# HicrestLaboratory/DLNetBench

Hardware: AMD Instinct MI355X
Metric: proxy iter time (ms) + effective GB/s, Llama-3-8B DP/FSDP at 1/2/4/8 MI355X (lower is better)
Workload: dtype bf16

## Files before the change

csrc/include/dlnb/kernels.hpp:

```cpp
#pragma once

#include <cstddef>
#include <cstdint>

#include "dlnb/common.hpp"

namespace dlnb {
namespace kernels {

void fill_random(void* p, size_t count, DType t, uint64_t seed, void* stream);

enum DlCounter : int {
  kCappedTasks = 0,
  kCappedTicks = 1,
  kWaitTimeouts = 2,
  kGateTimeouts = 3,
  kAbsorbedTicks = 4,
  kAbsorbedTasks = 5,
  kAborted = 6,
  kLateBlocks = 7,
  kNumCounters = 8
};
constexpr uint64_t kPoisonIter = ~0ull;
struct DlSync {
  uint64_t* tstart[2] = {nullptr, nullptr};
  const uint64_t* gate[2] = {nullptr, nullptr};
  uint32_t tag[2] = {0, 0};
  uint32_t chain = 0;
  uint64_t* counters = nullptr;
  const uint64_t* iter = nullptr;
  uint64_t gate_timeout = 0;
  uint64_t* done_gate = nullptr;
  uint32_t done_tag = 0;
  uint32_t pad = 0;
  const uint64_t* abort = nullptr;
};
constexpr uint32_t kTaskGateOnly = 1;
struct DlTask {
  DlSync sync;
  uint64_t ticks = 0;
  uint32_t epoch = 0;
  uint32_t work_rounds = 0;
  uint32_t tail_kt = 0;
  uint32_t flags = 0;
  uint64_t* tend = nullptr;
};
void gate_signal(uint64_t* gate, const uint64_t* iter, uint32_t tag, void* stream);
void fail_gate_signal(long index);
void gate_wait(const uint64_t* gate, const uint64_t* iter, uint32_t tag, uint64_t timeout_ticks, uint64_t* timeouts,
               void* stream, const uint64_t* abort = nullptr);
void set_word(uint64_t* word, uint64_t value, void* stream);
bool queues_independent(void* a, void* b, uint64_t timeout_ticks);

void idle_wait(uint64_t ticks, void* stream, uint64_t* start = nullptr, uint64_t* start2 = nullptr);
void busy_spin(uint64_t ticks, int blocks, void* stream, uint64_t* start = nullptr, uint64_t* start2 = nullptr);
double wallclock_hz(int device);
double wallclock_hz_nominal(int device);
double wallclock_uncertainty_ppm(int device);
void clock_cal_begin(int device);
void stamp(uint64_t* slot, void* stream);
void host_signal(uint64_t* word, uint64_t value, void* stream);
void lane_done(uint64_t* word, const uint64_t* iter, void* stream);
void host_wait(const uint64_t* word, uint64_t value, uint64_t timeout_ticks, uint64_t* timeouts, void* stream,
               uint64_t* iter_out = nullptr, uint64_t iter_value = 0, const uint64_t* abort = nullptr);
int num_cus(int device);

bool gemm_shape_ok(int M, int N, int K, DType in_t);
void gemm_tn(const void* A, const void* B, void* C, int M, int N, int K, int lda, int ldb, int ldc, DType in_t,
             void* stream, int variant = 0);
bool gemm_8phase_shape_ok(int M, int N, int K, DType in_t);
bool gemm_4wave_fp8_shape_ok(int M, int N, int K, DType in_t);
int gemm_group();
int gemm_narrow_nf(int M, int N, int cus);
bool gemm_tn_narrow(const void* A, const void* B, void* C, int M, int N, int K, int lda, int ldb, int ldc,
                    DType in_t, void* stream);
void gemm_tn_4wave_fp8(const void* A, const void* B, void* C, int M, int N, int K, int lda, int ldb, int ldc,
                       void* stream);
bool gemm_4wave_shape_ok(int M, int N, int K, DType in_t);
void gemm_tn_4wave_bf16(const void* A, const void* B, void* C, int M, int N, int K, int lda, int ldb, int ldc,
                        void* stream);
void gemm_tn_4wave_deadline(const void* A, const void* B, void* C, int M, int N, int K, DType in_t, uint64_t ticks,
                            uint64_t* slot, uint32_t epoch, int grid, void* stream, uint64_t slice_end,
                            const DlSync& sync);
void gemm_tn_4wave_fp8_deadline(const void* A, const void* B, void* C, int M, int N, int K, uint64_t ticks,
                                uint64_t* slot, uint32_t epoch, int grid, void* stream, uint64_t slice_end,
                                const DlSync& sync);
void gemm_tn_8phase(const void* A, const void* B, void* C, int M, int N, int K, int lda, int ldb, int ldc, DType in_t,
                    void* stream);
void gemm_tn_8phase_deadline(const void* A, const void* B, void* C, int M, int N, int K, DType in_t, uint64_t ticks,
                             uint64_t* slot, uint32_t epoch, int grid, void* stream, uint64_t slice_end,
                             const DlSync& sync);

void gemm_tn_deadline(const void* A, const void* B, void* C, int M, int N, int K, DType in_t, uint64_t ticks,
                      uint64_t* slot, uint32_t epoch, int grid, void* stream, uint64_t slice_end = 0,
                      const DlSync& sync = DlSync());

bool deadline_program_ok(int M, int N, int K, DType in_t);
void gemm_tn_deadline_program(const void* A, const void* B, void* C, int M, int N, int K, DType in_t,
                              const DlTask* tasks, int n, uint64_t* slot, int grid, void* stream,
                              uint32_t epoch = 0);
int program_ktiles(int M, int N, int K, DType in_t);
int program_tail_multiple(int M, int N, int K, DType in_t);

void sgd_momentum_bf16(void* param, void* mom, const void* grad, size_t n, float lr, float beta, void* stream,
                       uint64_t* end_stamp = nullptr, uint32_t* done = nullptr);

}
}
```

csrc/kernels/gemm_8phase.hip:

```cpp
#include <hip/hip_runtime.h>

#include <cstdlib>

#include "deadline_sync.hpp"
#include "dlnb/kernels.hpp"
#include "store_pair.hpp"

namespace dlnb {
namespace kernels {

namespace {

typedef __attribute__((ext_vector_type(8))) __bf16 bf16x8;
typedef __attribute__((ext_vector_type(4))) __bf16 bf16x4;
typedef __attribute__((ext_vector_type(4))) float f32x4;
typedef __attribute__((ext_vector_type(8))) int i32x8;
typedef __attribute__((ext_vector_type(4))) int i32x4;
typedef __attribute__((address_space(3))) void* lds_ptr_t;
typedef __attribute__((address_space(1))) void* gbl_ptr_t;

constexpr int kT = 256;
constexpr int kRB = 128;
constexpr int kHalf = 128 * kRB;
constexpr int kBuf = 4 * kHalf;
enum : int { kA0 = 0, kA1 = 1, kB0 = 2, kB1 = 3 };

__device__ __forceinline__ int swz(int row, int chunk) { return row * kRB + ((chunk ^ ((row >> 1) & 7)) << 4); }

template <int N>
__device__ __forceinline__ void wait_vm() {
  static_assert(N >= 0 && N < 64, "vmcnt range");
  __builtin_amdgcn_s_waitcnt((N & 15) | ((N >> 4) << 14) | (7 << 4) | (15 << 8));
}

__device__ __forceinline__ void raw_barrier() {
  __builtin_amdgcn_sched_barrier(0);
  __builtin_amdgcn_s_barrier();
  __builtin_amdgcn_sched_barrier(0);
}

__device__ __forceinline__ void stage_half(const char* base, int voff, size_t ld, int soff, char* lds, int w) {
  const __amdgpu_buffer_rsrc_t rs = __builtin_amdgcn_make_buffer_rsrc(const_cast<char*>(base), 0, 0x7ffffff0, 0x00020000);
#pragma unroll
  for (int i = 0; i < 2; ++i)
    __builtin_amdgcn_raw_ptr_buffer_load_lds(rs, (lds_ptr_t)(lds + (i * 8 + w) * 1024), 16, voff,
                                             soff + i * 64 * static_cast<int>(ld), 0, 0);
}

__device__ __forceinline__ int lane_offset(size_t ld, int w, int lane) {
  const int slot = w * 64 + lane;
  const int r = slot >> 3;
  const int q = (slot & 7) ^ ((r >> 1) & 7);
  return static_cast<int>(r * ld) + (q << 4);
}

__device__ __forceinline__ int xcd_remap(int b, int T) {
  const int q = T / 8, r = T % 8, x = b % 8;
  return (x < r ? x * (q + 1) : r * (q + 1) + (x - r) * q) + b / 8;
}

template <bool FP8>
struct Frags;
template <>
struct Frags<false> {
  bf16x8 a[2][4], bx[2][2], by[2][2];
};
template <>
struct Frags<true> {
  i32x8 a[4], bx[2], by[2];
};

template <bool FP8, int NF>
__device__ __forceinline__ void read_frags(const char* half, int row0, int r16, int h, bf16x8 (&f)[2][NF]) {
#pragma unroll
  for (int ks = 0; ks < 2; ++ks)
#pragma unroll
    for (int i = 0; i < NF; ++i) f[ks][i] = *reinterpret_cast<const bf16x8*>(half + swz(row0 + i * 16 + r16, ks * 4 + h));
}
template <bool FP8, int NF>
__device__ __forceinline__ void read_frags(const char* half, int row0, int r16, int h, i32x8 (&f)[NF]) {
#pragma unroll
  for (int i = 0; i < NF; ++i) {
    const int row = row0 + i * 16 + r16;
    const i32x4 lo = *reinterpret_cast<const i32x4*>(half + swz(row, h));
    const i32x4 hi = *reinterpret_cast<const i32x4*>(half + swz(row, h + 4));
    f[i] = __builtin_shufflevector(lo, hi, 0, 1, 2, 3, 4, 5, 6, 7);
  }
}

__device__ __forceinline__ void mfma_quadrant(f32x4 (&acc)[4][2], const bf16x8 (&a)[2][4], const bf16x8 (&b)[2][2]) {
#pragma unroll
  for (int ks = 0; ks < 2; ++ks)
#pragma unroll
    for (int i = 0; i < 4; ++i)
#pragma unroll
      for (int j = 0; j < 2; ++j) acc[i][j] = __builtin_amdgcn_mfma_f32_16x16x32_bf16(b[ks][j], a[ks][i], acc[i][j], 0, 0, 0);
}
__device__ __forceinline__ void mfma_quadrant(f32x4 (&acc)[4][2], const i32x8 (&a)[4], const i32x8 (&b)[2]) {
#pragma unroll
  for (int i = 0; i < 4; ++i)
#pragma unroll
    for (int j = 0; j < 2; ++j)
      acc[i][j] = __builtin_amdgcn_mfma_scale_f32_16x16x128_f8f6f4(b[j], a[i], acc[i][j], 0, 0, 0, 127, 0, 127);
}

struct Ctx {
  const char* Ab;
  const char* Bb;
  size_t lda, ldb;
  char* smem;
  int w, lane, wr, wc, r16, h;
  int last_kt;
  int voffA, voffB;
};

__device__ __forceinline__ void stage(const Ctx& c, int t, int slot) {
  const int tk = min(t, c.last_kt);
  const bool isA = slot == kA0 || slot == kA1;
  const int hi = slot == kA1 || slot == kB1;
  const char* base = isA ? c.Ab + static_cast<size_t>(hi) * 128 * c.lda : c.Bb + static_cast<size_t>(hi) * 128 * c.ldb;
  stage_half(base, isA ? c.voffA : c.voffB, isA ? c.lda : c.ldb, tk * kRB, c.smem + (t & 1) * kBuf + slot * kHalf, c.w);
}

typedef __attribute__((address_space(3))) volatile int lds_flag_t;
struct Deadline {
  uint64_t t0, ticks, slice_end;
  lds_flag_t* flag;
  int tid;
};

template <bool FP8, bool DL, bool BAL, int Q, int VM, bool STAGE, typename AF, typename BF>
__device__ __forceinline__ bool phase(const Ctx& c, int v, AF& fa, BF& b0r, BF& b1r, f32x4 (&acc)[2][2][4][2],
                                      const Deadline& d, uint64_t& now, bool has_next) {
  const char* cur = c.smem + (v & 1) * kBuf;
  if constexpr (Q == 0) {
    if constexpr (!BAL) {
      read_frags<FP8, 2>(cur + kB0 * kHalf, c.wc * 32, c.r16, c.h, b0r);
      __builtin_amdgcn_sched_barrier(0);
    }
    read_frags<FP8, 4>(cur + kA0 * kHalf, c.wr * 64, c.r16, c.h, fa);
  } else if constexpr (Q == 1) {
    read_frags<FP8, 2>(cur + kB1 * kHalf, c.wc * 32, c.r16, c.h, b1r);
  } else if constexpr (Q == 2) {
    read_frags<FP8, 4>(cur + kA1 * kHalf, c.wr * 64, c.r16, c.h, fa);
  } else {
    if constexpr (DL) {
      if (d.tid == 0) {
        const uint64_t el = (now - d.t0) & ((1ull << 48) - 1);
        d.flag[v & 1] = el >= d.ticks || el >= d.slice_end;
        asm volatile("s_waitcnt lgkmcnt(0)" ::: "memory");
      }
    }
    if constexpr (BAL) {
      if (has_next) read_frags<FP8, 2>(c.smem + ((v + 1) & 1) * kBuf + kB0 * kHalf, c.wc * 32, c.r16, c.h, b1r);
    }
  }
  if constexpr (STAGE) {
    if constexpr (Q == 0) stage(c, v + 1, kB1);
    if constexpr (Q == 1) stage(c, v + 1, kA1);
    if constexpr (Q == 2) stage(c, v + 2, BAL ? kB0 : kA0);
    if constexpr (Q == 3) stage(c, v + 2, BAL ? kA0 : kB0);
  }
  wait_vm<VM>();
  raw_barrier();
  int flag = 0;
  if constexpr (DL && Q == 3) flag = d.flag[v & 1];
  __builtin_amdgcn_sched_barrier(0);
  __builtin_amdgcn_s_setprio(1);
  if constexpr (Q == 0) mfma_quadrant(acc[0][0], fa, b0r);
  if constexpr (Q == 1) mfma_quadrant(acc[0][1], fa, b1r);
  if constexpr (Q == 2) mfma_quadrant(acc[1][1], fa, b1r);
  if constexpr (Q == 3) mfma_quadrant(acc[1][0], fa, b0r);
  __builtin_amdgcn_s_setprio(0);
  __builtin_amdgcn_sched_barrier(0);
  if constexpr (DL && Q == 2) now = __builtin_amdgcn_s_memrealtime();
  bool stop = false;
  if constexpr (DL && Q == 3) stop = __builtin_amdgcn_readfirstlane(flag) != 0;
  raw_barrier();
  return stop;
}

template <bool FP8, bool DL, bool BAL, int PAR, int V0, int V1, int V2, int V3, bool S01, bool S23>
__device__ __forceinline__ bool ktile(const Ctx& c, int v, Frags<FP8>& f, f32x4 (&acc)[2][2][4][2], const Deadline& d,
                                      bool has_next = true) {
  uint64_t now = 0;
  auto& b0r = (BAL && PAR == 1) ? f.by : f.bx;
  auto& b1r = (BAL && PAR == 1) ? f.bx : f.by;
  phase<FP8, DL, BAL, 0, V0, S01>(c, v, f.a, b0r, b1r, acc, d, now, has_next);
  phase<FP8, DL, BAL, 1, V1, S01>(c, v, f.a, b0r, b1r, acc, d, now, has_next);
  phase<FP8, DL, BAL, 2, V2, S23>(c, v, f.a, b0r, b1r, acc, d, now, has_next);
  return phase<FP8, DL, BAL, 3, V3, S23>(c, v, f.a, b0r, b1r, acc, d, now, has_next);
}

template <bool FP8, bool DL, bool BAL, int PAR>
__device__ __forceinline__ bool tail(const Ctx& c, int v, Frags<FP8>& f, f32x4 (&acc)[2][2][4][2], const Deadline& d) {
  if (ktile<FP8, DL, BAL, PAR, 8, 8, 6, 4, true, false>(c, v, f, acc, d)) return true;
  return ktile<FP8, DL, BAL, 1 - PAR, 2, 0, 0, 0, false, false>(c, v + 1, f, acc, d, false);
}

template <bool FP8, bool DL, bool BAL, bool UNI = false>
__device__ __forceinline__ bool tile(Ctx& c, const char* __restrict__ A, const char* __restrict__ B,
                                     __bf16* __restrict__ C, int M, int N, int K, int ldc, int b, const Deadline& d,
                                     int GROUP = 8) {
  const int nt_m = M / kT, nt_n = N / kT;
  const int per_group = GROUP * nt_n;
  const int first_m = (b / per_group) * GROUP;
  const int gsz = min(nt_m - first_m, GROUP);
  const int tm = first_m + (b % per_group) % gsz;
  const int tn = (b % per_group) / gsz;
  constexpr int esz = FP8 ? 1 : 2;
  c.Ab = A + static_cast<size_t>(tm) * kT * c.lda;
  c.Bb = B + static_cast<size_t>(tn) * kT * c.ldb;
  const int nk = (K * esz) / kRB;
  c.last_kt = UNI ? nk - 1 : 1 << 30;

  f32x4 acc[2][2][4][2];
#pragma unroll
  for (int qm = 0; qm < 2; ++qm)
#pragma unroll
    for (int qn = 0; qn < 2; ++qn)
#pragma unroll
      for (int i = 0; i < 4; ++i)
#pragma unroll
        for (int j = 0; j < 2; ++j) acc[qm][qn][i][j] = f32x4{0.f, 0.f, 0.f, 0.f};
  Frags<FP8> f;

  stage(c, 0, BAL ? kB0 : kA0);
  stage(c, 0, BAL ? kA0 : kB0);
  stage(c, 0, kB1);
  stage(c, 0, kA1);
  stage(c, 1, BAL ? kB0 : kA0);
  stage(c, 1, BAL ? kA0 : kB0);
  wait_vm<8>();
  raw_barrier();
  if constexpr (BAL) read_frags<FP8, 2>(c.smem + kB0 * kHalf, c.wc * 32, c.r16, c.h, f.bx);
  if (c.wr == 1) raw_barrier();

  bool stop = false;
  int v = 0;
  if constexpr (UNI) {
    if constexpr (!BAL) {
      for (; v < nk && !stop; ++v) stop = ktile<FP8, DL, false, 0, 8, 8, 8, 8, true, true>(c, v, f, acc, d);
    } else {
      for (; v < nk && !stop; v += 2) {
        stop = ktile<FP8, DL, true, 0, 8, 8, 8, 8, true, true>(c, v, f, acc, d);
        if (!stop) stop = ktile<FP8, DL, true, 1, 8, 8, 8, 8, true, true>(c, v + 1, f, acc, d);
      }
    }
    wait_vm<0>();
  } else if constexpr (!BAL) {
    for (; v < nk - 2 && !stop; ++v) stop = ktile<FP8, DL, false, 0, 8, 8, 8, 8, true, true>(c, v, f, acc, d);
    if (!stop) stop = tail<FP8, DL, false, 0>(c, v, f, acc, d);
  } else {
    for (; v < nk - 2 && !stop; v += 2) {
      stop = ktile<FP8, DL, true, 0, 8, 8, 8, 8, true, true>(c, v, f, acc, d);
      if (!stop) stop = ktile<FP8, DL, true, 1, 8, 8, 8, 8, true, true>(c, v + 1, f, acc, d);
    }
    if (!stop) stop = tail<FP8, DL, true, 0>(c, v, f, acc, d);
  }
  if (c.wr == 0) raw_barrier();
  if constexpr (DL) {
    if (stop) {
      wait_vm<0>();
      return false;
    }
  }

  const bool wide = epi::wide_ok(C, ldc);
#pragma unroll
  for (int qm = 0; qm < 2; ++qm)
#pragma unroll
    for (int qn = 0; qn < 2; ++qn)
#pragma unroll
      for (int i = 0; i < 4; ++i) {
        const int m = tm * kT + qm * 128 + c.wr * 64 + i * 16 + c.r16;
        const int n = tn * kT + qn * 128 + c.wc * 32;
        epi::store_pair<DL>(C + static_cast<size_t>(m) * ldc + n, acc[qm][qn][i][0], acc[qm][qn][i][1], c.h, wide);
      }
  return true;
}

template <bool FP8, bool DL, bool BAL = false, bool UNI = false>
__global__ void __launch_bounds__(512, 1)
    gemm_8phase_kernel(const char* __restrict__ A, const char* __restrict__ B, __bf16* __restrict__ C, int M, int N,
                       int K, int lda, int ldb, int ldc, uint64_t* __restrict__ slot, uint32_t epoch, uint64_t ticks,
                       uint64_t slice_end, DlSync sync, int group = 8, const DlTask* __restrict__ prog = nullptr,
                       int ntasks = 0) {
  __shared__ __attribute__((aligned(16))) char smem[2 * kBuf + 16];
  const int tid = threadIdx.x;
  Ctx c;
  c.lane = tid & 63;
  c.w = __builtin_amdgcn_readfirstlane(tid >> 6);
  c.wr = c.w >> 2;
  c.wc = c.w & 3;
  c.r16 = c.lane & 15;
  c.h = c.lane >> 4;
  c.smem = smem;
  constexpr int esz = FP8 ? 1 : 2;
  c.lda = static_cast<size_t>(lda) * esz;
  c.ldb = static_cast<size_t>(ldb) * esz;
  c.voffA = lane_offset(c.lda, c.w, c.lane);
  c.voffB = lane_offset(c.ldb, c.w, c.lane);
  const int T = (M / kT) * (N / kT);
  Deadline d{0, ticks, slice_end, (lds_flag_t*)(smem + 2 * kBuf), tid};
  if constexpr (!DL) {
    tile<FP8, false, BAL, UNI>(c, A, B, C, M, N, K, ldc, xcd_remap(blockIdx.x, T), d, group);
  } else {
    int round = 0;
    for (int k = 0;; ++k) {
      bool fixed = false;
      if (prog) {
        d.ticks = d.slice_end = prog[k].ticks;
        fixed = d.ticks == 0 && (prog[k].work_rounds | prog[k].tail_kt | prog[k].flags) != 0;
        if (d.ticks == 0 && !fixed) {
          if (blockIdx.x == 0 && tid == 0)
            for (int j = k; j < ntasks; ++j) dl::join(prog[j].sync);
          return;
        }
      }
      if (tid == 0) {
        if (prog) {
          const dl::ProgSeq ps = dl::program_seq(prog, k, epoch);
          d.t0 = dl::start_task(slot, ps.seq, ps.ep16, ps.mono, d.ticks, prog[k].sync, ps.it, k > 0).t0;
        } else {
          d.t0 = dl::agree_t0(slot, epoch, ticks, sync);
        }
      }
      if (fixed) {
        d.ticks = d.slice_end = 1ull << 48;
        const int rounds = static_cast<int>(prog[k].work_rounds);
        for (int r = 0; r < rounds; ++r, ++round)
          tile<FP8, true, BAL, UNI>(c, A, B, C, M, N, K, ldc, xcd_remap((blockIdx.x + round * gridDim.x) % T, T), d);
        const int tkt = static_cast<int>(prog[k].tail_kt);
        if (tkt > 0) {
          tile<FP8, true, BAL, UNI>(c, A, B, C, M, N, tkt * kRB / esz, ldc,
                                    xcd_remap((blockIdx.x + round * gridDim.x) % T, T), d);
          ++round;
        }
        if (tid == 0) dl::fixed_done(slot, prog[k].sync, prog[k].tend);
        if (k + 1 >= ntasks) return;
        continue;
      }
      if (prog && (prog[k].flags & kTaskGateOnly)) {
        dl::task_done(prog[k].sync);
// ... 46 lines not shown

struct StreamCtx {
  const char* A;
  const char* B;
  int nt_m, nt_n, T, nk;
  const char *Ab0, *Ab1, *Bb0, *Bb1;
};

__device__ __forceinline__ void stage_g(const Ctx& c, const StreamCtx& sc, int t, int base, int slot) {
  const int nxt = t - base >= sc.nk;
  const int kt = t - base - nxt * sc.nk;
  const bool isA = slot == kA0 || slot == kA1;
  const int hi = slot == kA1 || slot == kB1;
  const char* ab = nxt ? sc.Ab1 : sc.Ab0;
  const char* bb = nxt ? sc.Bb1 : sc.Bb0;
  const char* src = isA ? ab + static_cast<size_t>(hi) * 128 * c.lda : bb + static_cast<size_t>(hi) * 128 * c.ldb;
  stage_half(src, isA ? c.voffA : c.voffB, isA ? c.lda : c.ldb, kt * kRB, c.smem + (t & 1) * kBuf + slot * kHalf, c.w);
}

template <bool FP8, int Q, typename AF, typename BF>
__device__ __forceinline__ bool sphase(const Ctx& c, const StreamCtx& sc, int g, int base, bool after_store, AF& fa,
                                       BF& b0r, BF& b1r, f32x4 (&acc)[2][2][4][2], const Deadline& d, uint64_t& now) {
  const char* cur = c.smem + (g & 1) * kBuf;
  if constexpr (Q == 0) {
    read_frags<FP8, 2>(cur + kB0 * kHalf, c.wc * 32, c.r16, c.h, b0r);
    __builtin_amdgcn_sched_barrier(0);
    read_frags<FP8, 4>(cur + kA0 * kHalf, c.wr * 64, c.r16, c.h, fa);
  } else if constexpr (Q == 1) {
    read_frags<FP8, 2>(cur + kB1 * kHalf, c.wc * 32, c.r16, c.h, b1r);
  } else if constexpr (Q == 2) {
    read_frags<FP8, 4>(cur + kA1 * kHalf, c.wr * 64, c.r16, c.h, fa);
    now = __builtin_amdgcn_s_memrealtime();
  } else {
    if (d.tid == 0) {
      const uint64_t el = (now - d.t0) & ((1ull << 48) - 1);
      d.flag[g & 1] = el >= d.ticks || el >= d.slice_end;
      asm volatile("s_waitcnt lgkmcnt(0)" ::: "memory");
    }
  }
  if constexpr (Q == 0) stage_g(c, sc, g + 1, base, kB1);
  if constexpr (Q == 1) stage_g(c, sc, g + 1, base, kA1);
  if constexpr (Q == 2) stage_g(c, sc, g + 2, base, kA0);
  if constexpr (Q == 3) stage_g(c, sc, g + 2, base, kB0);
  if (after_store)
    wait_vm<40>();
  else
    wait_vm<8>();
  raw_barrier();
  bool stop = false;
  if constexpr (Q == 3) stop = __builtin_amdgcn_readfirstlane(d.flag[g & 1]) != 0;
  __builtin_amdgcn_s_setprio(1);
  if constexpr (Q == 0) mfma_quadrant(acc[0][0], fa, b0r);
  if constexpr (Q == 1) mfma_quadrant(acc[0][1], fa, b1r);
  if constexpr (Q == 2) mfma_quadrant(acc[1][1], fa, b1r);
  if constexpr (Q == 3) mfma_quadrant(acc[1][0], fa, b0r);
  __builtin_amdgcn_s_setprio(0);
  raw_barrier();
  return stop;
}

template <bool FP8>
__device__ __forceinline__ bool sktile(const Ctx& c, const StreamCtx& sc, int g, int base, bool after_store,
                                       Frags<FP8>& f, f32x4 (&acc)[2][2][4][2], const Deadline& d) {
  uint64_t now = 0;
  sphase<FP8, 0>(c, sc, g, base, after_store, f.a, f.bx, f.by, acc, d, now);
  sphase<FP8, 1>(c, sc, g, base, after_store, f.a, f.bx, f.by, acc, d, now);
  sphase<FP8, 2>(c, sc, g, base, after_store, f.a, f.bx, f.by, acc, d, now);
  return sphase<FP8, 3>(c, sc, g, base, after_store, f.a, f.bx, f.by, acc, d, now);
}

template <bool FP8>
__global__ void __launch_bounds__(512, 1)
    gemm_8phase_stream_kernel(const char* __restrict__ A, const char* __restrict__ B, __bf16* __restrict__ C, int M,
                              int N, int K, int lda, int ldb, int ldc, uint64_t* __restrict__ slot, uint32_t epoch,
                              uint64_t ticks, uint64_t slice_end, DlSync sync) {
  __shared__ __attribute__((aligned(16))) char smem[2 * kBuf + 16];
  const int tid = threadIdx.x;
  Ctx c;
  c.lane = tid & 63;
  c.w = __builtin_amdgcn_readfirstlane(tid >> 6);
  c.wr = c.w >> 2;
  c.wc = c.w & 3;
  c.r16 = c.lane & 15;
  c.h = c.lane >> 4;
  c.smem = smem;
  constexpr int esz = FP8 ? 1 : 2;
  c.lda = static_cast<size_t>(lda) * esz;
  c.ldb = static_cast<size_t>(ldb) * esz;
  c.voffA = lane_offset(c.lda, c.w, c.lane);
  c.voffB = lane_offset(c.ldb, c.w, c.lane);
  Deadline d{0, ticks, slice_end, (lds_flag_t*)(smem + 2 * kBuf), tid};
  if (tid == 0) d.t0 = dl::agree_t0(slot, epoch, ticks, sync);
  StreamCtx sc;
  sc.A = A;
  sc.B = B;
  sc.nt_m = M / kT;
  sc.nt_n = N / kT;
  sc.T = sc.nt_m * sc.nt_n;
  sc.nk = (K * esz) / kRB;
  int tm0, tn0, tm1, tn1;
  int round = 0;
  tile_coords(xcd_remap(blockIdx.x % sc.T, sc.T), sc.nt_m, sc.nt_n, tm0, tn0);
  tile_coords(xcd_remap((blockIdx.x + gridDim.x) % sc.T, sc.T), sc.nt_m, sc.nt_n, tm1, tn1);
  sc.Ab0 = A + static_cast<size_t>(tm0) * kT * c.lda;
  sc.Bb0 = B + static_cast<size_t>(tn0) * kT * c.ldb;
  sc.Ab1 = A + static_cast<size_t>(tm1) * kT * c.lda;
  sc.Bb1 = B + static_cast<size_t>(tn1) * kT * c.ldb;

  f32x4 acc[2][2][4][2];
#pragma unroll
  for (int qm = 0; qm < 2; ++qm)
#pragma unroll
    for (int qn = 0; qn < 2; ++qn)
#pragma unroll
      for (int i = 0; i < 4; ++i)
#pragma unroll
        for (int j = 0; j < 2; ++j) acc[qm][qn][i][j] = f32x4{0.f, 0.f, 0.f, 0.f};
  Frags<FP8> f;

  stage_g(c, sc, 0, 0, kA0);
  stage_g(c, sc, 0, 0, kB0);
  stage_g(c, sc, 0, 0, kB1);
  stage_g(c, sc, 0, 0, kA1);
  stage_g(c, sc, 1, 0, kA0);
  stage_g(c, sc, 1, 0, kB0);
  wait_vm<8>();
  raw_barrier();
  if (c.wr == 1) raw_barrier();

  int g = 0;
  int base = 0;
  bool stop = false;
  while (!stop) {
    stop = sktile<FP8>(c, sc, g, base, g == base && base > 0, f, acc, d);
    ++g;
    if (!stop && g == base + sc.nk) {
      store_tile<FP8>(c, C, ldc, tm0, tn0, acc);
      base = g;
      ++round;
      tm0 = tm1;
      tn0 = tn1;
      sc.Ab0 = sc.Ab1;
      sc.Bb0 = sc.Bb1;
      tile_coords(xcd_remap((blockIdx.x + (round + 1) * gridDim.x) % sc.T, sc.T), sc.nt_m, sc.nt_n, tm1, tn1);
      sc.Ab1 = A + static_cast<size_t>(tm1) * kT * c.lda;
      sc.Bb1 = B + static_cast<size_t>(tn1) * kT * c.ldb;
    }
  }
  wait_vm<0>();
  if (c.wr == 0) raw_barrier();
  dl::task_done(sync);
}

}

bool gemm_8phase_shape_ok(int M, int N, int K, DType in_t) {
  const size_t esz = dtype_size(in_t);
  return gemm_shape_ok(M, N, K, in_t) && (static_cast<size_t>(K) * esz) / kRB >= 2;
}

void gemm_tn_8phase(const void* A, const void* B, void* C, int M, int N, int K, int lda, int ldb, int ldc, DType in_t,
                    void* stream) {
  DLNB_REQUIRE(gemm_8phase_shape_ok(M, N, K, in_t), "gemm 8-phase: unsupported shape M=" << M << " N=" << N << " K=" << K);
  const int tiles = (M / kT) * (N / kT);
  const int group = gemm_group();
  hipStream_t st = static_cast<hipStream_t>(stream);
  auto* a = static_cast<const char*>(A);
  auto* b = static_cast<const char*>(B);
  auto* cc = static_cast<__bf16*>(C);
  const bool even = (static_cast<size_t>(K) * dtype_size(in_t) / kRB) % 2 == 0;
  if (in_t == DType::FP8_E4M3) {
    hipLaunchKernelGGL((gemm_8phase_kernel<true, false, false, true>), tiles, 512, 0, st, a, b, cc, M, N, K, lda, ldb,
                       ldc, nullptr, 0u, 0ull, 0ull, DlSync(), group);
  } else if (even) {
    hipLaunchKernelGGL((gemm_8phase_kernel<false, false, true>), tiles, 512, 0, st, a, b, cc, M, N, K, lda, ldb, ldc,
                       nullptr, 0u, 0ull, 0ull, DlSync(), group);
  } else {
    hipLaunchKernelGGL((gemm_8phase_kernel<false, false>), tiles, 512, 0, st, a, b, cc, M, N, K, lda, ldb, ldc, nullptr,
                       0u, 0ull, 0ull, DlSync(), group);
  }
  hipError_t e = hipGetLastError();
  if (e != hipSuccess) DLNB_THROW("gemm 8-phase launch failed: " << hipGetErrorString(e));
}

static int deadline_group() {
  const char* env = std::getenv("DLNB_DEADLINE_GROUP");
  const int g = env ? std::atoi(env) : 0;
  return g > 0 ? g : 8;
}

bool deadline_program_8phase_ok(int M, int N, int K, DType in_t) {
  return gemm_8phase_shape_ok(M, N, K, in_t);
}

void gemm_8phase_deadline_program(const void* A, const void* B, void* C, int M, int N, int K, DType in_t,
                                  const DlTask* tasks, int n, uint64_t* slot, int grid, void* stream, uint32_t epoch) {
  DLNB_REQUIRE(deadline_program_8phase_ok(M, N, K, in_t), "gemm 8-phase deadline program: unsupported shape");
  DLNB_REQUIRE(tasks != nullptr && n > 0 && slot != nullptr && grid > 0, "gemm 8-phase deadline program: bad args");
  hipStream_t st = static_cast<hipStream_t>(stream);
  auto* a = static_cast<const char*>(A);
  auto* b = static_cast<const char*>(B);
  auto* cc = static_cast<__bf16*>(C);
  const int nk = static_cast<int>(static_cast<size_t>(K) * dtype_size(in_t) / kRB);
  const DlSync none;
  if (in_t == DType::BF16 && nk % 2 == 0)
    hipLaunchKernelGGL((gemm_8phase_kernel<false, true, true>), grid, 512, 0, st, a, b, cc, M, N, K, K, K, N, slot,
                       epoch, 0ull, 0ull, none, deadline_group(), tasks, n);
  else if (in_t == DType::BF16)
    hipLaunchKernelGGL((gemm_8phase_kernel<false, true>), grid, 512, 0, st, a, b, cc, M, N, K, K, K, N, slot, epoch,
                       0ull, 0ull, none, deadline_group(), tasks, n);
  else
    hipLaunchKernelGGL((gemm_8phase_kernel<true, true, false, true>), grid, 512, 0, st, a, b, cc, M, N, K, K, K, N,
                       slot, epoch, 0ull, 0ull, none, deadline_group(), tasks, n);
  hipError_t e = hipGetLastError();
  if (e != hipSuccess) DLNB_THROW("gemm 8-phase deadline program launch failed: " << hipGetErrorString(e));
}

void gemm_tn_8phase_deadline(const void* A, const void* B, void* C, int M, int N, int K, DType in_t, uint64_t ticks,
                             uint64_t* slot, uint32_t epoch, int grid, void* stream, uint64_t slice_end,
                             const DlSync& sync) {
  DLNB_REQUIRE(gemm_8phase_shape_ok(M, N, K, in_t), "gemm 8-phase deadline: unsupported shape");
  hipStream_t st = static_cast<hipStream_t>(stream);
  auto* a = static_cast<const char*>(A);
  auto* b = static_cast<const char*>(B);
  auto* cc = static_cast<__bf16*>(C);
  const int nk = static_cast<int>(static_cast<size_t>(K) * dtype_size(in_t) / kRB);
  if (in_t == DType::BF16 && nk <= 16) {
    hipLaunchKernelGGL((gemm_8phase_stream_kernel<false>), grid, 512, 0, st, a, b, cc, M, N, K, K, K, N, slot, epoch,
                       ticks, slice_end, sync);
  } else if (in_t == DType::BF16 && nk % 2 == 0) {
    hipLaunchKernelGGL((gemm_8phase_kernel<false, true, true>), grid, 512, 0, st, a, b, cc, M, N, K, K, K, N, slot,
                       epoch, ticks, slice_end, sync, deadline_group());
  } else if (in_t == DType::BF16) {
    hipLaunchKernelGGL((gemm_8phase_kernel<false, true>), grid, 512, 0, st, a, b, cc, M, N, K, K, K, N, slot, epoch,
                       ticks, slice_end, sync, deadline_group());
  } else {
    hipLaunchKernelGGL((gemm_8phase_kernel<true, true, false, true>), grid, 512, 0, st, a, b, cc, M, N, K, K, K, N, slot,
                       epoch, ticks, slice_end, sync, deadline_group());
  }
  hipError_t e = hipGetLastError();
  if (e != hipSuccess) DLNB_THROW("gemm 8-phase deadline launch failed: " << hipGetErrorString(e));
}

}
}
```

csrc/src/compute.cpp:

```cpp
#include "dlnb/compute.hpp"

#include <algorithm>
#include <cmath>
#include <exception>
#include <map>
#include <set>

#include "dlnb/kernels.hpp"
#include "dlnb/timers.hpp"

namespace dlnb {

ComputeMode parse_compute_mode(const std::string& s, DeviceKind dev) {
  if (s == "auto") return dev == DeviceKind::GPU ? ComputeMode::Gemm : ComputeMode::Sleep;
  if (s == "sleep") return ComputeMode::Sleep;
  if (s == "spin") return ComputeMode::Spin;
  if (s == "gemm") return ComputeMode::Gemm;
  if (s == "gemm-work" || s == "gemm_work") return ComputeMode::GemmWork;
  if (s == "flops") return ComputeMode::Flops;
  DLNB_THROW("unknown compute mode '" << s << "' (auto, sleep, spin, gemm, flops)");
}

const char* compute_mode_name(ComputeMode m) {
  switch (m) {
// ... 384 lines not shown
      j["deadline_slice_us"] = slice_us_;
      j["chained_tasks"] = chained_;
      j["chain_absorb_us"] = absorb_ticks_ / hz() * 1e6;
      j["gated_tasks"] = gated_;
      j["programs"] = programs_launched_;
      j["program_tasks"] = program_tasks_;
    }
    if (A_.data()) {
      j["gemm_dtype"] = dtype_name(dtype_);
      j["gemm_N"] = N_;
      j["gemm_K"] = K_;
    }
    if (fixed_) {
      Json f = Json::object();
      f["round_us"] = cal_.round_us;
      f["ktile_us"] = cal_.ktile_us;
      f["grid"] = grid_;
      f["ktiles_per_tile"] = nk_;
      f["tflops"] = round_flops() / (cal_.round_us * 1e-6) / 1e12;
      f["tasks"] = fixed_tasks_;
      f["calibration"] = cal_given_ ? "DLNB_FIXED_WORK_CAL" : "measured";
      j["fixed_work"] = f;
    }
    return j;
  }
  ComputeMode mode() const override { return mode_; }
  bool product(const void** c, size_t* count, DType* t) const override {
    if (!C_.data()) return false;
    *c = C_.data();
    *count = static_cast<size_t>(kMmax) * N_;
    *t = DType::BF16;
    return true;
  }

 private:
  uint64_t ticks(double us) const { return static_cast<uint64_t>(us * 1e-6 * hz() + 0.5); }
  double hz() const {
    if (hz_ <= 0.0) hz_ = kernels::wallclock_hz(dev_.index());
    return hz_;
  }

  const kernels::DlTask* place_tasks(Stream& s, const std::vector<kernels::DlTask>& ts) {
    const size_t n = ts.size();
    DLNB_REQUIRE(n <= kProgTasks, "compute program of " << n << " tasks exceeds the ring (" << kProgTasks << ")");
    if (dev_.capturing(s)) {
      if (prog_next_ + n > kProgTasks) prog_next_ = 0;
      kernels::DlTask* dst = prog_dev_.as<kernels::DlTask>() + prog_next_;
      prog_next_ += n;
      uploads_.push_back(Upload{dst, ts});
      return dst;
    }
    if (host_next_ + n > kProgTasks) host_next_ = 0;
    kernels::DlTask* dst = prog_host_ + host_next_;
    host_next_ += n;
    std::copy(ts.begin(), ts.end(), dst);
    __atomic_thread_fence(__ATOMIC_SEQ_CST);
    return dst;
  }

  void deadline_task(Stream& s, double d, kernels::DlSync sync, bool chain, Event* done = nullptr) {
    uint64_t* slot = slot_for(s);
    sync.chain = chain ? absorb_ticks_ : 0u;
    sync.counters = counters_.as<uint64_t>();
    sync.iter = dev_.iter_word();
    sync.gate_timeout = gate_timeout_ticks_;
    sync.abort = dev_.abort_word();
    uint64_t* dgate = nullptr;
    uint32_t dtag = 0;
    const bool folded = done && dev_.arm_gate_record(*done, s, &dgate, &dtag);
    const uint64_t total = ticks(d);
    auto pit = programs_.find(&s);
    if (pit != programs_.end() && pit->second.open) {
      DLNB_REQUIRE(folded || !done, "a program task's done event needs gate events");
      kernels::DlTask t;
      t.sync = sync;
      t.sync.done_gate = dgate;
      t.sync.done_tag = dtag;
      t.ticks = total;
      take_pending(s, pit->second, t.sync);
      DLNB_REQUIRE(pit->second.index < 4096, "more than 4096 program tasks per iteration on one stream");
      t.epoch = pit->second.index++;
      pit->second.tasks.push_back(t);
      pit->second.done_free = t.sync.done_gate == nullptr;
      chain_live_[slot] = true;
      return;
    }
    const uint32_t ep = next_epoch(slot);
    const uint64_t slice = slice_us_ > 0 ? std::max<uint64_t>(ticks(slice_us_), 1) : total;
    for (uint64_t end = slice;; end += slice) {
      kernels::DlSync ls = end == slice ? sync : kernels::DlSync();
      ls.abort = sync.abort;
      if (end >= total && folded) {
        ls.done_gate = dgate;
        ls.done_tag = dtag;
        ls.iter = sync.iter;
      }
      kernels::gemm_tn_deadline(A_.data(), B_.data(), C_.data(), kMmax, N_, K_, dtype_, total, slot, ep, grid_,
                                s.native(), std::min(end, total), ls);
      if (end >= total) break;
    }
    if (done && !folded) s.record(*done);
    chain_live_[slot] = true;
  }

  uint32_t next_epoch(uint64_t* slot) {
    uint32_t& ep0 = epoch_[slot];
    ep0 = ep0 % 32767 + 1;
    return 32767 + ep0;
  }

  double round_flops() const { return static_cast<double>(grid_) * 2.0 * kTile * kTile * K_; }
  FixedWork size_work(double us, double flops) const {
    FixedWork w;
    double units;
    if (mode_ == ComputeMode::Flops)
      units = std::max(0.0, flops * scale_) / round_flops();
    else
      units = std::max(0.0, us * scale_) / cal_.round_us;
    w.rounds = static_cast<uint32_t>(std::floor(units));
    const double kt = (units - w.rounds) * nk_;
    uint32_t tail = static_cast<uint32_t>(std::lround(kt / tail_mul_)) * tail_mul_;
    if (tail >= static_cast<uint32_t>(nk_)) {
      ++w.rounds;
      tail = 0;
    }
    w.tail_kt = tail;
    if (w.rounds == 0 && w.tail_kt == 0 && units > 0) w.tail_kt = tail_mul_;
    w.us = w.rounds * cal_.round_us + w.tail_kt * cal_.ktile_us;
    return w;
  }

  void fixed_task(Stream& s, double us, double flops, uint64_t* start, kernels::DlSync sync, Event* done) {
    const FixedWork w = size_work(us, flops);
    note_task(s, w.us);
    if (stall_timers_ && !start) start = stall_timers_->slot();
    uint64_t* end = stall_timers_ ? stall_timers_->slot() : nullptr;
    sync.tstart[0] = start;
    sync.tstart[1] = extra_start_;
    extra_start_ = nullptr;
    sync.counters = counters_.as<uint64_t>();
    sync.iter = dev_.iter_word();
    sync.gate_timeout = gate_timeout_ticks_;
    sync.abort = dev_.abort_word();
    uint64_t* dgate = nullptr;
    uint32_t dtag = 0;
    const bool folded = done && dev_.arm_gate_record(*done, s, &dgate, &dtag);
    sync.done_gate = dgate;
    sync.done_tag = dtag;
    kernels::DlTask t;
    t.sync = sync;
    t.ticks = 0;
    t.work_rounds = w.rounds;
    t.tail_kt = w.tail_kt;
    t.tend = end;
    auto pit = programs_.find(&s);
    if (pit != programs_.end() && pit->second.open) {
      DLNB_REQUIRE(folded || !done, "a program task's done event needs gate events");
      take_pending(s, pit->second, t.sync);
      DLNB_REQUIRE(pit->second.index < 4096, "more than 4096 program tasks per iteration on one stream");
      t.epoch = pit->second.index++;
      pit->second.tasks.push_back(t);
      pit->second.done_free = t.sync.done_gate == nullptr;
    } else {
      for (int i = 0; i < 2; ++i)
        if (t.sync.gate[i])
          kernels::gate_wait(t.sync.gate[i], dev_.iter_word(), t.sync.tag[i], gate_timeout_ticks_,
                             counters_.as<uint64_t>() + kernels::kWaitTimeouts, s.native(), dev_.abort_word());
      uint64_t* slot = slot_for(s);
      const kernels::DlTask* dst = place_tasks(s, {t});
      kernels::gemm_tn_deadline_program(A_.data(), B_.data(), C_.data(), kMmax, N_, K_, dtype_, dst, 1, slot, grid_,
                                        s.native(), next_epoch(slot));
      if (done && !folded) s.record(*done);
    }
    ++fixed_tasks_;
    if (end) last_end_[&s] = end;
    if (stall_timers_) stall_timers_->task_started(s, start, 0, end);
    if (task_timers_ && start && end) {
      task_timers_->pair(start, end, "compute_task_time");
      task_timers_->add("compute_task_table", (mode_ == ComputeMode::Flops ? w.us : us * scale_) * 1e-6);
    }
  }

  uint64_t* slot_for(Stream& s) {
    auto it = slot_of_.find(&s);
    size_t idx;
    if (it == slot_of_.end()) {
      idx = slot_of_.size();
      DLNB_REQUIRE(idx < kSlots, "too many compute streams");
      slot_of_[&s] = idx;
    } else {
      idx = it->second;
    }
    return slots_.as<uint64_t>() + idx * 8;
  }

  void alloc_operands() {
    const int Mmax = kMmax;
    const size_t esz = dtype_size(dtype_);
    A_ = dev_.alloc(static_cast<size_t>(Mmax) * K_ * esz);
    B_ = dev_.alloc(static_cast<size_t>(N_) * K_ * esz);
    C_ = dev_.alloc(static_cast<size_t>(Mmax) * N_ * 2);
    auto s = dev_.create_stream(false);
    dev_.fill_random(A_.data(), static_cast<size_t>(Mmax) * K_, dtype_, 1, *s);
    dev_.fill_random(B_.data(), static_cast<size_t>(N_) * K_, dtype_, 2, *s);
    dev_.memset_async(C_.data(), 0, C_.bytes(), *s);
    s->synchronize();
  }

  void calibrate() {
    nk_ = kernels::program_ktiles(kMmax, N_, K_, dtype_);
    tail_mul_ = static_cast<uint32_t>(std::max(1, kernels::program_tail_multiple(kMmax, N_, K_, dtype_)));
    const std::string given = env_or("DLNB_FIXED_WORK_CAL", "");
    if (!given.empty()) {
      const auto kv = split(trim(given), ':');
      DLNB_REQUIRE(kv.size() == 2, "DLNB_FIXED_WORK_CAL: expected round_us:ktile_us, got '" << given << "'");
      cal_.round_us = std::stod(kv[0]);
      cal_.ktile_us = std::stod(kv[1]);
      DLNB_REQUIRE(cal_.round_us > 0 && cal_.ktile_us > 0, "DLNB_FIXED_WORK_CAL: bad values '" << given << "'");
      cal_given_ = true;
      return;
    }
    auto s = dev_.create_stream(false);
    auto e0 = dev_.create_event(true);
    auto e1 = dev_.create_event(true);
    uint64_t* slot = slot_for(*s);
    auto time_task = [&](uint32_t rounds, uint32_t tail) {
      kernels::DlTask t;
      t.sync.counters = counters_.as<uint64_t>();
      t.sync.abort = dev_.abort_word();
      t.work_rounds = rounds;
      t.tail_kt = tail;
      const kernels::DlTask* dst = place_tasks(*s, {t});
      s->record(*e0);
      kernels::gemm_tn_deadline_program(A_.data(), B_.data(), C_.data(), kMmax, N_, K_, dtype_, dst, 1, slot, grid_,
                                        s->native(), next_epoch(slot));
      s->record(*e1);
      s->synchronize();
      return dev_.elapsed_ms(*e0, *e1) * 1e3;
    };
    const double probe = std::max(1.0, time_task(8, 0) / 8.0);
    const uint32_t warm = static_cast<uint32_t>(std::min(4000.0, std::max(20.0, 300000.0 / probe)));
    (void)time_task(warm, 0);
    auto best = [&](uint32_t r, uint32_t tail) {
      double b = 1e30;
      for (int i = 0; i < 3; ++i) b = std::min(b, time_task(r, tail));
      return b;
    };
    const uint32_t r1 = 20, r2 = 60;
    const double t1 = best(r1, 0), t2 = best(r2, 0);
    cal_.round_us = std::max(1e-3, (t2 - t1) / (r2 - r1));
    const uint32_t tail = std::max<uint32_t>(tail_mul_, static_cast<uint32_t>(nk_ / 2) / tail_mul_ * tail_mul_);
    const double tt = best(r1, tail);
    cal_.ktile_us = std::max(1e-4, (tt - t1) / tail);
    dev_.memset_async(slot, 0, 64, *s);
    s->synchronize();
    slot_of_.clear();
    epoch_.clear();
  }

  static constexpr int kMmax = 8192;
  static constexpr int kTile = 256;
  static constexpr size_t kSlots = 64;
  Device& dev_;
  ComputeMode mode_;
  double scale_;
  bool fixed_ = false;
  Buffer slots_;
  Buffer counters_;
  struct Fold : Device::StreamFold {
    GpuCompute* e = nullptr;
    Stream* s = nullptr;
    void fold_wait(const uint64_t* gate, uint32_t tag) override { e->fold_wait(*s, gate, tag); }
    void fold_record(Event& ev) override { e->fold_record(*s, ev); }
  };
  struct Program {
    bool open = false;
    uint32_t index = 0;
    std::vector<kernels::DlTask> tasks;
    std::vector<std::pair<const uint64_t*, uint32_t>> pending;
    bool done_free = false;
    bool split = false;
    Fold fold;
  };

  void fold_wait(Stream& s, const uint64_t* gate, uint32_t tag) {
    Program& p = programs_[&s];
    for (auto& w : p.pending)
      if (w.first == gate) {
        w.second = tag;
        return;
      }
    p.pending.emplace_back(gate, tag);
  }
  void fold_record(Stream& s, Event& ev) {
    Program& p = programs_[&s];
    uint64_t* g = nullptr;
    uint32_t tag = 0;
    DLNB_REQUIRE(dev_.arm_gate_record(ev, s, &g, &tag), "fold_record: not a gate event");
    if (p.pending.empty() && p.done_free && !p.tasks.empty()) {
      p.tasks.back().sync.done_gate = g;
      p.tasks.back().sync.done_tag = tag;
      p.done_free = false;
      return;
    }
    emit_pending(s, p, g, tag);
    if (p.tasks.empty() || p.tasks.back().sync.done_gate != g) {
      kernels::DlTask t = gate_task();
      t.sync.done_gate = g;
      t.sync.done_tag = tag;
      push_task(p, t);
    }
    p.done_free = false;
  }
  kernels::DlTask gate_task() const {
    kernels::DlTask t;
    t.sync.iter = dev_.iter_word();
    t.sync.counters = counters_.as<uint64_t>();
    t.sync.gate_timeout = gate_timeout_ticks_;
    t.sync.abort = dev_.abort_word();
    t.ticks = fixed_ ? 0 : 1;
    t.flags = kernels::kTaskGateOnly;
    return t;
  }
  void push_task(Program& p, const kernels::DlTask& t) {
    DLNB_REQUIRE(p.index < 4096, "more than 4096 program tasks per iteration on one stream");
    kernels::DlTask c = t;
    c.epoch = p.index++;
    p.tasks.push_back(c);
  }
  void emit_pending(Stream& s, Program& p, uint64_t* done_gate, uint32_t done_tag) {
    (void)s;
    while (!p.pending.empty()) {
      kernels::DlTask t = gate_task();
      for (int i = 0; i < 2 && !p.pending.empty(); ++i) {
        t.sync.gate[i] = p.pending.front().first;
        t.sync.tag[i] = p.pending.front().second;
        p.pending.erase(p.pending.begin());
      }
      if (p.pending.empty() && done_gate) {
        t.sync.done_gate = done_gate;
        t.sync.done_tag = done_tag;
      }
      push_task(p, t);
      p.done_free = false;
    }
  }
  void take_pending(Stream& s, Program& p, kernels::DlSync& sync) {
    if (p.pending.empty()) return;
    const size_t free_slots = (sync.gate[0] ? 0u : 1u) + (sync.gate[1] ? 0u : 1u);
    if (p.pending.size() > free_slots) {
      std::vector<std::pair<const uint64_t*, uint32_t>> keep(p.pending.end() - static_cast<long>(free_slots),
                                                             p.pending.end());
      p.pending.resize(p.pending.size() - free_slots);
      emit_pending(s, p, nullptr, 0);
      p.pending = keep;
    }
    for (int i = 0; i < 2 && !p.pending.empty(); ++i) {
      if (sync.gate[i]) continue;
      sync.gate[i] = p.pending.front().first;
      sync.tag[i] = p.pending.front().second;
      p.pending.erase(p.pending.begin());
    }
  }
  std::map<Stream*, Program> programs_;
  struct Join {
    std::vector<uint64_t*> gates;
    uint32_t tag;
    uint64_t* host_done;
  };
  std::map<Stream*, Join> joins_;
  std::set<Stream*> joined_;
  std::map<Stream*, long> program_count_;
  Buffer prog_dev_;
  size_t prog_next_ = 0;
  kernels::DlTask* prog_host_ = nullptr;
  size_t host_next_ = 0;
  struct Upload {
    kernels::DlTask* dst;
    std::vector<kernels::DlTask> tasks;
  };
  std::vector<Upload> uploads_;
  static constexpr size_t kProgTasks = 16384;
  long programs_launched_ = 0, program_tasks_ = 0, fixed_tasks_ = 0;
  std::vector<uint64_t*> gates_;
// ... 56 lines not shown
```

Before: 2815.

## Add streaming 8-phase GEMM program kernel prefetching next tile across boundaries

Adds a new BF16 deadline-program kernel that streams consecutive output tiles and stages the next tile's first k-tiles into LDS while the current tile finishes. This hides the prologue and drain bubble between tiles in fixed-work GEMM tasks. Fixed tasks are now marked with a flag so work_rounds=0 tasks with a tail are still recognised. The change adds complexity in the wait counts after a store and may alter how calibration maps rounds to time.

```diff
diff --git a/csrc/include/dlnb/kernels.hpp b/csrc/include/dlnb/kernels.hpp
--- a/csrc/include/dlnb/kernels.hpp
+++ b/csrc/include/dlnb/kernels.hpp
@@ -36,6 +36,7 @@
   const uint64_t* abort = nullptr;
 };
 constexpr uint32_t kTaskGateOnly = 1;
+constexpr uint32_t kTaskFixed = 2;
 struct DlTask {
   DlSync sync;
   uint64_t ticks = 0;
diff --git a/csrc/kernels/gemm_8phase.hip b/csrc/kernels/gemm_8phase.hip
--- a/csrc/kernels/gemm_8phase.hip
+++ b/csrc/kernels/gemm_8phase.hip
@@ -112,6 +112,10 @@
   int w, lane, wr, wc, r16, h;
   int last_kt;
   int voffA, voffB;
+  const char* Ab1;
+  const char* Bb1;
+  int nk;
+  bool after_store;
 };
 
 __device__ __forceinline__ void stage(const Ctx& c, int t, int slot) {
@@ -122,6 +126,17 @@
   stage_half(base, isA ? c.voffA : c.voffB, isA ? c.lda : c.ldb, tk * kRB, c.smem + (t & 1) * kBuf + slot * kHalf, c.w);
 }
 
+__device__ __forceinline__ void stage_next(const Ctx& c, int t, int slot) {
+  const bool nxt = t >= c.nk;
+  const int tk = nxt ? t - c.nk : t;
+  const bool isA = slot == kA0 || slot == kA1;
+  const int hi = slot == kA1 || slot == kB1;
+  const char* ab = nxt ? c.Ab1 : c.Ab;
+  const char* bb = nxt ? c.Bb1 : c.Bb;
+  const char* base = isA ? ab + static_cast<size_t>(hi) * 128 * c.lda : bb + static_cast<size_t>(hi) * 128 * c.ldb;
+  stage_half(base, isA ? c.voffA : c.voffB, isA ? c.lda : c.ldb, tk * kRB, c.smem + (t & 1) * kBuf + slot * kHalf, c.w);
+}
+
 typedef __attribute__((address_space(3))) volatile int lds_flag_t;
 struct Deadline {
   uint64_t t0, ticks, slice_end;
@@ -129,7 +144,8 @@
   int tid;
 };
 
-template <bool FP8, bool DL, bool BAL, int Q, int VM, bool STAGE, typename AF, typename BF>
+template <bool FP8, bool DL, bool BAL, int Q, int VM, bool STAGE, bool STREAM = false, int VMA = VM, typename AF,
+          typename BF>
 __device__ __forceinline__ bool phase(const Ctx& c, int v, AF& fa, BF& b0r, BF& b1r, f32x4 (&acc)[2][2][4][2],
                                       const Deadline& d, uint64_t& now, bool has_next) {
   const char* cur = c.smem + (v & 1) * kBuf;
@@ -155,13 +171,25 @@
       if (has_next) read_frags<FP8, 2>(c.smem + ((v + 1) & 1) * kBuf + kB0 * kHalf, c.wc * 32, c.r16, c.h, b1r);
     }
   }
-  if constexpr (STAGE) {
+  if constexpr (STAGE && STREAM) {
+    if constexpr (Q == 0) stage_next(c, v + 1, kB1);
+    if constexpr (Q == 1) stage_next(c, v + 1, kA1);
+    if constexpr (Q == 2) stage_next(c, v + 2, BAL ? kB0 : kA0);
+    if constexpr (Q == 3) stage_next(c, v + 2, BAL ? kA0 : kB0);
+  } else if constexpr (STAGE) {
     if constexpr (Q == 0) stage(c, v + 1, kB1);
     if constexpr (Q == 1) stage(c, v + 1, kA1);
     if constexpr (Q == 2) stage(c, v + 2, BAL ? kB0 : kA0);
     if constexpr (Q == 3) stage(c, v + 2, BAL ? kA0 : kB0);
   }
-  wait_vm<VM>();
+  if constexpr (VMA != VM) {
+    if (c.after_store)
+      wait_vm<VMA>();
+    else
+      wait_vm<VM>();
+  } else {
+    wait_vm<VM>();
+  }
   raw_barrier();
   int flag = 0;
   if constexpr (DL && Q == 3) flag = d.flag[v & 1];
@@ -190,6 +218,18 @@
   phase<FP8, DL, BAL, 1, V1, S01>(c, v, f.a, b0r, b1r, acc, d, now, has_next);
   phase<FP8, DL, BAL, 2, V2, S23>(c, v, f.a, b0r, b1r, acc, d, now, has_next);
   return phase<FP8, DL, BAL, 3, V3, S23>(c, v, f.a, b0r, b1r, acc, d, now, has_next);
+}
+
+template <int PAR, int VMA>
+__device__ __forceinline__ bool sktile_bal(const Ctx& c, int v, Frags<false>& f, f32x4 (&acc)[2][2][4][2],
+                                           const Deadline& d) {
+  uint64_t now = 0;
+  auto& b0r = PAR == 1 ? f.by : f.bx;
+  auto& b1r = PAR == 1 ? f.bx : f.by;
+  phase<false, true, true, 0, 8, true, true, VMA>(c, v, f.a, b0r, b1r, acc, d, now, true);
+  phase<false, true, true, 1, 8, true, true, VMA>(c, v, f.a, b0r, b1r, acc, d, now, true);
+  phase<false, true, true, 2, 8, true, true, VMA>(c, v, f.a, b0r, b1r, acc, d, now, true);
+  return phase<false, true, true, 3, 8, true, true, VMA>(c, v, f.a, b0r, b1r, acc, d, now, true);
 }
 
 template <bool FP8, bool DL, bool BAL, int PAR>
@@ -542,6 +582,118 @@
   dl::task_done(sync);
 }
 
+__device__ __forceinline__ bool stream_tile(Ctx& c, __bf16* __restrict__ C, int ldc, int tm, int tn, bool primed,
+                                            Frags<false>& f, f32x4 (&acc)[2][2][4][2], const Deadline& d) {
+  if (!primed) {
+#pragma unroll
+    for (int qm = 0; qm < 2; ++qm)
+#pragma unroll
+      for (int qn = 0; qn < 2; ++qn)
+#pragma unroll
+        for (int i = 0; i < 4; ++i)
+#pragma unroll
+          for (int j = 0; j < 2; ++j) acc[qm][qn][i][j] = f32x4{0.f, 0.f, 0.f, 0.f};
+    stage_next(c, 0, kB0);
+    stage_next(c, 0, kA0);
+    stage_next(c, 0, kB1);
+    stage_next(c, 0, kA1);
+    stage_next(c, 1, kB0);
+    stage_next(c, 1, kA0);
+    wait_vm<8>();
+    raw_barrier();
+    read_frags<false, 2>(c.smem + kB0 * kHalf, c.wc * 32, c.r16, c.h, f.bx);
+    if (c.wr == 1) raw_barrier();
+  }
+  c.after_store = primed;
+  bool stop = sktile_bal<0, 24>(c, 0, f, acc, d);
+  if (!stop) stop = sktile_bal<1, 8>(c, 1, f, acc, d);
+  for (int v = 2; v < c.nk && !stop; v += 2) {
+    stop = sktile_bal<0, 8>(c, v, f, acc, d);
+    if (!stop) stop = sktile_bal<1, 8>(c, v + 1, f, acc, d);
+  }
+  if (stop) return false;
+  store_tile<false>(c, C, ldc, tm, tn, acc);
+  return true;
+}
+
+__device__ __forceinline__ void stream_tile_at(const Ctx& c, const char* A, const char* B, int idx, int nt_m, int nt_n,
+                                               int& tm, int& tn, const char*& ab, const char*& bb) {
+  const int T = nt_m * nt_n;
+  tile_coords(xcd_remap(idx % T, T), nt_m, nt_n, tm, tn);
+  ab = A + static_cast<size_t>(tm) * kT * c.lda;
+  bb = B + static_cast<size_t>(tn) * kT * c.ldb;
+}
+
+__device__ __forceinline__ void stream_drain(const Ctx& c) {
+  wait_vm<0>();
+  if (c.wr == 0) raw_barrier();
+}
+
+__global__ void __launch_bounds__(512, 1)
+    gemm_8phase_stream_program_kernel(const char* __restrict__ A, const char* __restrict__ B, __bf16* __restrict__ C,
+                                      int M, int N, int K, uint64_t* __restrict__ slot, uint32_t epoch,
+                                      const DlTask* __restrict__ prog, int ntasks) {
+  __shared__ __attribute__((aligned(16))) char smem[2 * kBuf + 16];
+  const int tid = threadIdx.x;
+  Ctx c;
+  c.lane = tid & 63;
+  c.w = __builtin_amdgcn_readfirstlane(tid >> 6);
+  c.wr = c.w >> 2;
+  c.wc = c.w & 3;
+  c.r16 = c.lane & 15;
+  c.h = c.lane >> 4;
+  c.smem = smem;
+  c.lda = c.ldb = static_cast<size_t>(K) * 2;
+  c.voffA = lane_offset(c.lda, c.w, c.lane);
+  c.voffB = lane_offset(c.ldb, c.w, c.lane);
+  c.last_kt = 1 << 30;
+  const int nt_m = M / kT, nt_n = N / kT;
+  const int nk_full = (K * 2) / kRB;
+  Deadline d{0, 0, 0, (lds_flag_t*)(smem + 2 * kBuf), tid};
+  f32x4 acc[2][2][4][2];
+  Frags<false> f;
+  int round = 0, tm, tn, tm1, tn1;
+  for (int k = 0;; ++k) {
+    d.ticks = d.slice_end = prog[k].ticks;
+    const bool fixed = d.ticks == 0 && (prog[k].work_rounds | prog[k].tail_kt | prog[k].flags) != 0;
+    if (d.ticks == 0 && !fixed) {
+      if (blockIdx.x == 0 && tid == 0)
+        for (int j = k; j < ntasks; ++j) dl::join(prog[j].sync);
+      return;
+    }
+    if (tid == 0) {
+      const dl::ProgSeq ps = dl::program_seq(prog, k, epoch);
+      d.t0 = dl::start_task(slot, ps.seq, ps.ep16, ps.mono, d.ticks, prog[k].sync, ps.it, k > 0).t0;
+    }
+    int rounds = 1 << 30, total = 1 << 30, tkt = 0;
+    if (fixed) {
+      d.ticks = d.slice_end = 1ull << 48;
+      rounds = static_cast<int>(prog[k].work_rounds);
+      tkt = static_cast<int>(prog[k].tail_kt);
+      total = rounds + (tkt > 0 ? 1 : 0);
+    }
+    if (prog[k].flags & kTaskGateOnly) total = 0;
+    for (int i = 0; i < total; ++i) {
+      stream_tile_at(c, A, B, blockIdx.x + round * gridDim.x, nt_m, nt_n, tm, tn, c.Ab, c.Bb);
+      c.nk = i < rounds ? nk_full : tkt;
+      c.Ab1 = c.Ab;
+      c.Bb1 = c.Bb;
+      if (i + 1 < total)
+        stream_tile_at(c, A, B, blockIdx.x + (round + 1) * gridDim.x, nt_m, nt_n, tm1, tn1, c.Ab1, c.Bb1);
+      const bool stored = stream_tile(c, C, N, tm, tn, i > 0, f, acc, d);
+      ++round;
+      if (!stored) break;
+    }
+    if (total > 0) stream_drain(c);
+    if (fixed) {
+      if (tid == 0) dl::fixed_done(slot, prog[k].sync, prog[k].tend);
+    } else {
+      dl::task_done(prog[k].sync);
+    }
+    if (k + 1 >= ntasks) return;
+  }
+}
+
 }
 
 bool gemm_8phase_shape_ok(int M, int N, int K, DType in_t) {
@@ -594,8 +746,7 @@
   const int nk = static_cast<int>(static_cast<size_t>(K) * dtype_size(in_t) / kRB);
   const DlSync none;
   if (in_t == DType::BF16 && nk % 2 == 0)
-    hipLaunchKernelGGL((gemm_8phase_kernel<false, true, true>), grid, 512, 0, st, a, b, cc, M, N, K, K, K, N, slot,
-                       epoch, 0ull, 0ull, none, deadline_group(), tasks, n);
+    hipLaunchKernelGGL(gemm_8phase_stream_program_kernel, grid, 512, 0, st, a, b, cc, M, N, K, slot, epoch, tasks, n);
   else if (in_t == DType::BF16)
     hipLaunchKernelGGL((gemm_8phase_kernel<false, true>), grid, 512, 0, st, a, b, cc, M, N, K, K, K, N, slot, epoch,
                        0ull, 0ull, none, deadline_group(), tasks, n);
diff --git a/csrc/src/compute.cpp b/csrc/src/compute.cpp
--- a/csrc/src/compute.cpp
+++ b/csrc/src/compute.cpp
@@ -560,6 +560,7 @@
     t.ticks = 0;
     t.work_rounds = w.rounds;
     t.tail_kt = w.tail_kt;
+    t.flags = kernels::kTaskFixed;
     t.tend = end;
     auto pit = programs_.find(&s);
     if (pit != programs_.end() && pit->second.open) {
@@ -638,6 +639,7 @@
       t.sync.abort = dev_.abort_word();
       t.work_rounds = rounds;
       t.tail_kt = tail;
+      t.flags = kernels::kTaskFixed;
       const kernels::DlTask* dst = place_tasks(*s, {t});
       s->record(*e0);
       kernels::gemm_tn_deadline_program(A_.data(), B_.data(), C_.data(), kMmax, N_, K_, dtype_, dst, 1, slot, grid_,
```

Measured after the change: 2815. Within noise of the previous version (+0.0%).
